# tsdconseil/libtsd

Hardware: AMD Instinct MI355X
Metric: Msamples/s, 127-tap FIR on 2^26 cfloat stream (higher is better)
Workload: dtype f32 (complex64 data, real f32 taps); 1 GPU; configs[1]: 127-tap FIR (design_rif_fen lp 0.02, real taps via filtrer()) on 2^26-sample Veccf per GPU, inputs resident in HBM; method=overlap-save, samples_per_gpu=67108864, pre_warm_steps=150, backend=none (one process, one GPU), world_size=1, self_launched=False

## Files before the change

### libtsd_amd/csrc/ols.hip

```cpp
#include "fir_internal.hpp"
#include "fft1024_wave.hpp"
#include <cstdlib>

namespace tsdgpu {

using namespace w1024;
constexpr int OLS_N = 1024;
#ifndef OLS_SCALAR
#define OLS_SCALAR 1
#endif
#ifndef OLS_RUN_DEFAULT
#define OLS_RUN_DEFAULT 2
#endif
#ifndef OLS_DYN_DEFAULT
#define OLS_DYN_DEFAULT 16
#endif
constexpr int OLS_MAX_CTR = 32;
#if OLS_SCALAR
using cv = cpx;
#else
using cv = v2f;
#endif
__device__ __forceinline__ cv mkv(float a, float b) { return Make<cv>::of(a, b); }

constexpr bool NT = false;
__device__ __forceinline__ cv ntload(const cv *p)
{
  v2f t = __builtin_nontemporal_load(reinterpret_cast<const v2f *>(p));
  return mkv(t.x, t.y);
}
__device__ __forceinline__ void ntstore(cv *p, cv v)
{
  v2f t = {v.x, v.y};
  __builtin_nontemporal_store(t, reinterpret_cast<v2f *>(p));
}
template <bool EDGE>
__device__ __forceinline__ void ols_fetch_real(cv (&v)[16], const float *__restrict__ x, const float *__restrict__ hist,
                                               int histlen, int Km1, int L, int64_t n, int64_t b, int lane)
{
  const int64_t ga = 2 * b * (int64_t) L - Km1, gb = ga + L;
  if (!EDGE) {
    const float *xa = x + ga, *xb = x + gb;
#pragma unroll
    for (int r = 0; r < 16; r++) v[r] = mkv(xa[64 * r + lane], xb[64 * r + lane]);
  } else {
#pragma unroll
    for (int r = 0; r < 16; r++) {
      const int64_t g1 = ga + 64 * r + lane, g2 = gb + 64 * r + lane;
      v[r] = mkv(g1 < 0 ? hist[histlen + g1] : (g1 < n ? x[g1] : 0.f), g2 < 0 ? hist[histlen + g2] : (g2 < n ? x[g2] : 0.f));
    }
  }
}
template <bool EDGE>
__device__ __forceinline__ void ols_fetch(cv (&v)[16], const cv *__restrict__ x, const cv *__restrict__ hist,
                                          int histlen, int Km1, int L, int64_t n, int64_t b, int lane)
{
  const int64_t g0 = b * (int64_t) L - Km1;
  if (!EDGE) {
    const cv *xb = x + g0;
#pragma unroll
    for (int r = 0; r < 16; r++) v[r] = NT ? ntload(xb + 64 * r + lane) : xb[64 * r + lane];
  } else {
#pragma unroll
    for (int r = 0; r < 16; r++) {
      const int64_t g = g0 + 64 * r + lane;
      v[r] = g < 0 ? hist[histlen + g] : (g < n ? x[g] : mkv(0.f, 0.f));
    }
  }
}

struct OlsDyn {
  unsigned *ctr;
  unsigned base, Q;
  int NC;
  int64_t nunits;
};
struct RegTab {
  cv v[16];
  __device__ __forceinline__ const cv &operator[](int r) const { return v[r]; }
};

template <bool EDGE, bool REAL, int R0, bool DYN>
__device__ __forceinline__ void ols_body(cv *lds, const void *__restrict__ xv, const void *__restrict__ histv,
                                         void *__restrict__ yv, const cv *__restrict__ Hreg,
                                         const cv *__restrict__ TW1, const cv *__restrict__ TW2, int Km1,
                                         int histlen, int L, int64_t n, int64_t b_lo, int64_t b_hi, int64_t G,
                                         int64_t w, int64_t cgrp, int R, OlsDyn dyn)
{
  const int lane = threadIdx.x & 63;
  const cv *x = (const cv *) xv, *hist = (const cv *) histv;
  cv *y = (cv *) yv;
  const float *xr = (const float *) xv, *histr = (const float *) histv;
  float *yr = (float *) yv;
  RegTab tw1r, tw2r, Hr;
#pragma unroll
  for (int r = 0; r < 16; r++) {
    tw1r.v[r] = TW1[r * 64 + lane];
    tw2r.v[r] = TW2[r * 64 + lane];
    Hr.v[r] = Hreg[r * 64 + lane];
  }
  auto sync = []() {
    __builtin_amdgcn_fence(__ATOMIC_RELEASE, "wavefront");
    __builtin_amdgcn_wave_barrier();
    __builtin_amdgcn_fence(__ATOMIC_ACQUIRE, "wavefront");
  };

  const int64_t slot = (G % 8 == 0) ? (w % 8) * (G / 8) + w / 8 : w;
  const int ctr_c = DYN ? (int) (cgrp % dyn.NC) : 0;
  auto pull_issue = [&]() -> unsigned {
    unsigned v = 0;
    if (lane == 0) v = __hip_atomic_fetch_add(dyn.ctr + ctr_c * 32, 1u, __ATOMIC_RELAXED, __HIP_MEMORY_SCOPE_AGENT);
    return v;
  };
  auto pull = [&]() -> int64_t {
    for (;;) {
      const unsigned v = (unsigned) __builtin_amdgcn_readfirstlane((int) pull_issue()) - dyn.base;
      if (v >= dyn.Q) return -1;
      const int64_t u = (int64_t) v * dyn.NC + ctr_c;
      if (u < dyn.nunits) return u;
    }
  };
  auto pull_finish = [&](unsigned raw) -> int64_t {
    const unsigned v = (unsigned) __builtin_amdgcn_readfirstlane((int) raw) - dyn.base;
    if (v >= dyn.Q) return -1;
    const int64_t u = (int64_t) v * dyn.NC + ctr_c;
    return u < dyn.nunits ? u : pull();
  };
  int64_t unit = EDGE ? 0 : (DYN ? pull() : slot);
  if (unit < 0) return;
  int64_t run0 = EDGE ? b_lo : b_lo + unit * R;
  int64_t b = run0;
  if (b >= b_hi) return;

  int64_t pulled = -1;
  auto process = [&](cv (&cur)[16], cv (&nxt)[16], int64_t blk, int64_t nb, bool inrun) {
    const bool more = !EDGE && nb < b_hi;
    cv keep[R0 > 0 ? R0 : 1], pre[R0 > 0 ? R0 : 1];
#pragma unroll
    for (int r = 0; r < R0; r++) keep[r] = cur[(16 - R0 + r) & 15];
    const int64_t pb = more ? nb : blk;
    if (!EDGE && R0 > 0) {
      if (!REAL) {
        const cv *xb = x + (pb * (int64_t) L - Km1);
        if (!inrun) {
#pragma unroll
          for (int r = 0; r < R0; r++) pre[r] = xb[64 * r + lane];
        }
#pragma unroll
        for (int r = R0; r < 16; r++) nxt[r] = NT ? ntload(xb + 64 * r + lane) : xb[64 * r + lane];
      } else {
        const float *xa = xr + (2 * pb * (int64_t) L - Km1), *xb = xa + L;
        if (!inrun) {
#pragma unroll
          for (int r = 0; r < R0; r++) pre[r] = mkv(xa[64 * r + lane], xb[64 * r + lane]);
        }
#pragma unroll
        for (int r = R0; r < 16; r++) nxt[r] = mkv(xa[64 * r + lane], xb[64 * r + lane]);
      }
    } else if (!EDGE) {
      if (REAL) ols_fetch_real<EDGE>(nxt, xr, histr, histlen, Km1, L, n, pb, lane);
      else ols_fetch<EDGE>(nxt, x, hist, histlen, Km1, L, n, pb, lane);
    }
    const bool pulls = DYN && more && !inrun;
    unsigned raw = 0;
    if (pulls) raw = pull_issue();
    forward(cur, lds, lane, tw1r, tw2r, sync);
#pragma unroll
    for (int r = 0; r < 16; r++) cur[r] = cmul(cur[r], Hr[r]);
    inverse(cur, lds, lane, tw1r, tw2r, sync);
    sync();
    if (!EDGE) {
#pragma unroll
      for (int r = R0; r < 16; r++) asm volatile("" ::"v"(nxt[r]));
#pragma unroll
      for (int r = 0; r < R0; r++) {
        asm volatile("" : "+v"(keep[r]));
        if (inrun) nxt[r] = REAL ? mkv(keep[r].y, nxt[(16 - R0 + r) & 15].x) : keep[r];
        else nxt[r] = pre[r];
      }
    }
    if (pulls) pulled = pull_finish(raw);
    const int r0 = (!EDGE && R0 > 0) ? R0 : Km1 >> 6;
    if (!REAL) {
      const int64_t o0 = blk * (int64_t) L;
      cv *yb = y + (o0 - Km1);
#pragma unroll
      for (int r = 0; r < 16; r++) {
        const int t = 64 * r + lane;
        if (!EDGE) {
          if (r >= r0) { if (NT) ntstore(yb + t, cur[r]); else yb[t] = cur[r]; }
        } else {
          if (r >= r0 && o0 + t - Km1 < n) yb[t] = cur[r];
        }
      }
    } else {
      const int64_t oa = 2 * blk * (int64_t) L, ob = oa + L;
      float *ya = yr + (oa - Km1), *yb = yr + (ob - Km1);
#pragma unroll
      for (int r = 0; r < 16; r++) {
        const int t = 64 * r + lane;
        if (!EDGE) {
          if (r >= r0) { ya[t] = cur[r].x; yb[t] = cur[r].y; }
        } else {
          if (r >= r0 && oa + t - Km1 < n) ya[t] = cur[r].x;
          if (r >= r0 && ob + t - Km1 < n) yb[t] = cur[r].y;
        }
      }
    }
  };

  cv A[16], B[16];
  if (REAL) ols_fetch_real<EDGE>(A, xr, histr, histlen, Km1, L, n, b, lane);
  else ols_fetch<EDGE>(A, x, hist, histlen, Km1, L, n, b, lane);
  if (EDGE) {
    process(A, B, b, b_hi, false);
    return;
  }
#pragma unroll
  for (int r = 0; r < 16; r++) asm volatile("" ::"v"(A[r]));
  int i = 0;
  constexpr int64_t END = INT64_MAX;
  auto unit_after = [&](int64_t u) -> int64_t {
    if (DYN) return pulled;
    return b_lo + (u + G) * R < b_hi ? u + G : -1;
  };
  int64_t unit_next = DYN ? pull() : unit_after(unit);
  auto next_of = [&](int64_t &nb, bool &inrun) {
    inrun = i + 1 < R && b + 1 < b_hi;
    nb = inrun ? b + 1 : (unit_next >= 0 ? b_lo + unit_next * R : END);
  };
  auto advance = [&](int64_t nb, bool inrun) {
    if (inrun) i++;
    else {
      i = 0;
      run0 = nb;
      unit = unit_next;
      unit_next = unit_after(unit);
    }
    b = nb;
  };
  for (;;) {
    int64_t nb;
    bool inrun;
    next_of(nb, inrun);
    process(A, B, b, nb, inrun);
    if (nb >= b_hi) break;
    advance(nb, inrun);
    next_of(nb, inrun);
    process(B, A, b, nb, inrun);
    if (nb >= b_hi) break;
    advance(nb, inrun);
  }
}

template <bool REAL, int R0, bool DYN>
__global__ __launch_bounds__(64, 2) void ols_kernel(const void *__restrict__ x, const void *__restrict__ hist,
                                                    void *__restrict__ hist_next, void *__restrict__ y,
                                                    const cpx *__restrict__ Hreg, const cpx *__restrict__ TW1,
                                                    const cpx *__restrict__ TW2, int Km1, int histlen, int L,
                                                    int64_t n, int64_t b_lo, int64_t b_hi, int64_t nblocks, int G,
                                                    int ne, int64_t n_lo, int64_t b_tail, int R, OlsDyn dyn)
{
  __shared__ cv lds[LDS_ELEMS];
  const int64_t w = (int64_t) blockIdx.x;
  const int lane = threadIdx.x & 63;
  if (w < G) {
    ols_body<false, REAL, R0, DYN>(lds, x, hist, y, (const cv *) Hreg, (const cv *) TW1, (const cv *) TW2, Km1, histlen, L, n, b_lo, b_hi, G,
                                       w, (int64_t) blockIdx.x / 8, R, dyn);
  } else if (w < G + ne) {
    const int64_t b = (w - G) < n_lo ? (int64_t) (w - G) : b_tail + (w - G - n_lo);
    ols_body<true, REAL, 0, false>(lds, x, hist, y, (const cv *) Hreg, (const cv *) TW1, (const cv *) TW2, Km1, histlen, L, n, b, nblocks, 1, 0, 0, 1, dyn);
  } else if (w == G + ne) {
    for (int i = lane; i < histlen; i += 64) {
      const int64_t g = n - histlen + i;
      if (REAL) ((float *) hist_next)[i] = g < 0 ? ((const float *) hist)[histlen + g] : ((const float *) x)[g];
      else ((cpx *) hist_next)[i] = g < 0 ? ((const cpx *) hist)[histlen + g] : ((const cpx *) x)[g];
    }
  }
}

bool ols_preferred(const tsdgpu_fir *f)
{
  if (ols_long_supported(f)) return true;
  if (f->data_type == TSDGPU_C64) return f->K >= (f->tap_type == TSDGPU_F32 ? 57 : 48) && f->K <= 513;
  return f->tap_type == TSDGPU_F32 && f->K >= 40 && f->K <= 513;
}

int ols_plan_create(tsdgpu_fir *f)
{
  if (ols_long_supported(f)) return ols_long_plan_create(f);
  if (f->K > OLS_N - 63) {
    f->method = TSDGPU_FIR_DIRECT;
    return TSDGPU_OK;
  }
  const int N = OLS_N, K = f->K;
  f->ols_N = N;
  f->ols_L = N - (int) (cdiv(K - 1, 64) * 64);
  std::vector<double> hr(K), hi(K, 0.0);
  if (f->tap_type == TSDGPU_F32) {
    const float *t = (const float *) f->taps_host.data();
    for (int i = 0; i < K; i++) hr[i] = t[i];
  } else {
    const float *t = (const float *) f->taps_host.data();
    for (int i = 0; i < K; i++) { hr[i] = t[2 * i]; hi[i] = t[2 * i + 1]; }
  }
  struct Tables {
    std::vector<double> c, s;
    std::vector<cpx> tw12;
    Tables() : c(OLS_N / 2), s(OLS_N / 2), tw12(2 * OLS_N)
    {
      const double PI = 3.14159265358979323846;
      for (int i = 0; i < OLS_N / 2; i++) { c[i] = std::cos(2 * PI * i / OLS_N); s[i] = -std::sin(2 * PI * i / OLS_N); }
      fill_twiddles(tw12.data(), tw12.data() + OLS_N);
    }
  };
  static const Tables *tb = new Tables();
  std::vector<double> ar(N, 0.0), ai(N, 0.0);
  int logn = 0;
  while ((1 << logn) < N) logn++;
  for (int i = 0; i < K; i++) {
    int rv = 0;
    for (int b = 0; b < logn; b++) rv |= ((i >> b) & 1) << (logn - 1 - b);
    ar[rv] = hr[i];
    ai[rv] = hi[i];
  }
  for (int len = 2; len <= N; len <<= 1) {
    const int half = len / 2, step = N / len;
    for (int base = 0; base < N; base += len)
      for (int j = 0; j < half; j++) {
        const double wr = tb->c[(size_t) j * step], wi = tb->s[(size_t) j * step];
        const int a = base + j, b = a + half;
        const double tr = ar[b] * wr - ai[b] * wi, ti = ar[b] * wi + ai[b] * wr;
        ar[b] = ar[a] - tr; ai[b] = ai[a] - ti;
        ar[a] += tr; ai[a] += ti;
      }
  }
  std::vector<cpx> img(3 * (size_t) N);
  for (int lane = 0; lane < 64; lane++)
    for (int r = 0; r < 16; r++) {
      const int k = freq_index(lane, r);
      img[r * 64 + lane] = mk((float) (ar[k] / N), (float) (ai[k] / N));
    }
  std::copy(tb->tw12.begin(), tb->tw12.end(), img.begin() + N);
  const size_t bytes = (size_t) N * sizeof(cpx);
  const size_t ctr_bytes = (size_t) OLS_MAX_CTR * 128;
  img.resize(3 * (size_t) N + ctr_bytes / sizeof(cpx), mk(0.f, 0.f));
  if (hipMalloc(&f->d_H, 3 * bytes + ctr_bytes) != hipSuccess)
    return set_err(TSDGPU_ERR_HIP, "ols: hipMalloc failed: %s", hipGetErrorString(hipGetLastError()));
  if (hipMemcpy(f->d_H, img.data(), 3 * bytes + ctr_bytes, hipMemcpyHostToDevice) != hipSuccess)
    return set_err(TSDGPU_ERR_HIP, "ols: upload failed: %s", hipGetErrorString(hipGetLastError()));
  f->d_ctr = (unsigned *) ((char *) f->d_H + 3 * bytes);
  f->ctr_base = 0;
  static const std::pair<int, int> occ = []() {
    int dev = 0, cus = 256, per_cu = 8;
    (void) hipGetDevice(&dev);
    (void) hipDeviceGetAttribute(&cus, hipDeviceAttributeMultiprocessorCount, dev);
    if (hipOccupancyMaxActiveBlocksPerMultiprocessor(&per_cu, ols_kernel<false, 2, true>, 64, 0) != hipSuccess || per_cu < 1) {
      (void) hipGetLastError();
      per_cu = 8;
    }
    return std::make_pair(cus, per_cu);
  }();
  const int cus = occ.first, per_cu = occ.second;
  f->ols_grid = cus * per_cu;
  if (getenv("TSDGPU_DEBUG")) fprintf(stderr, "[tsdgpu] ols plan: N=%d K=%d L=%d cus=%d waves/CU=%d grid=%d waves\n", N, K, f->ols_L, cus, per_cu, f->ols_grid);
  return TSDGPU_OK;
}

void ols_plan_destroy(tsdgpu_fir *f)
{
  if (f->d_H) (void) hipFree(f->d_H);
  f->d_H = nullptr;
  f->d_ctr = nullptr;
}

int ols_step(tsdgpu_fir *f, const void *x, void *y, int64_t n, hipStream_t st)
{
  const bool real = f->data_type == TSDGPU_F32;
  const int L = f->ols_L;
  const int64_t LB = real ? 2 * (int64_t) L : L;
  const int64_t nblocks = cdiv(n, LB);
  const cpx *d = (const cpx *) f->d_H;
  const int64_t ovl = OLS_N - L;
  const int64_t b_lo = std::min<int64_t>(nblocks, f->K > 1 ? cdiv(ovl, LB) : 0);
  const int64_t b_hi = std::max<int64_t>(b_lo, n / LB);
  int64_t grid = 0;
  const int r0 = (int) (ovl / 64);
  const char *run_s = dev_switch("OLS_RUN");
  const int run_env = run_s ? atoi(run_s) : OLS_RUN_DEFAULT;
  const char *nc_s = dev_switch("OLS_DYN");
  int NC = nc_s ? atoi(nc_s) : OLS_DYN_DEFAULT;
  if (NC < 0 || NC > OLS_MAX_CTR || f->capturable || !f->d_ctr || stream_is_capturing(st)) NC = 0;
  int R = 1;
  unsigned ctr_add = 0;
  OlsDyn dyn = {f->d_ctr, f->ctr_base, 0u, NC > 0 ? NC : 1, 0};
  if (b_hi > b_lo) {
    const int64_t nint = b_hi - b_lo;
    if (r0 >= 1 && r0 <= 4 && run_env > 1 && nint >= (int64_t) f->ols_grid * run_env * 2) R = run_env;
    const int64_t nruns = cdiv(nint, R);
    const char *min_s = dev_switch("OLS_DYN_MIN");
    const int64_t dyn_min = min_s ? atoi(min_s) : 4;
    if (NC > 0 && nruns >= dyn_min * (int64_t) f->ols_grid) {
      const int64_t grp = (int64_t) 8 * NC;
      grid = std::max<int64_t>(grp, (f->ols_grid / grp) * grp);
      if (NC != f->ctr_nc) {
        TSD_HIP(hipMemsetAsync(f->d_ctr, 0, (size_t) OLS_MAX_CTR * 128, st));
        f->ctr_base = 0;
        f->ctr_nc = NC;
        dyn.base = 0;
      }
      dyn.nunits = nruns;
      dyn.Q = (unsigned) cdiv(nruns, NC);
      ctr_add = dyn.Q + (unsigned) (grid / NC);
    } else {
      NC = 0;
      grid = nruns < f->ols_grid ? nruns : f->ols_grid;
      if (nruns > grid) {
        const int64_t rounds = cdiv(nruns, grid);
        grid = cdiv(cdiv(nruns, rounds), 8) * 8;
      }
    }
  } else NC = 0;
  const int64_t b_lo_w = b_lo;
  const int64_t n_lo = b_lo, b_tail = b_hi;
  const int ne = (int) (n_lo + (nblocks - b_tail));
  int64_t e[2] = {n_lo, b_tail};
  const int nxt = f->cur ^ 1;
  const unsigned nwg = (unsigned) (grid + ne + 1);
#define OLS_LAUNCH(REAL, R0, DYN)                                                                                                     \
  hipLaunchKernelGGL((ols_kernel<REAL, R0, DYN>), dim3(nwg), dim3(64), 0, st, x, (const void *) fir_hist_read(f),                        \
                     f->hist[nxt], y, d, d + OLS_N, d + 2 * OLS_N, OLS_N - L, f->HL, L, n, b_lo_w, b_hi, nblocks, (int) grid, ne,   \
                     e[0], e[1], R, dyn)
#define OLS_LAUNCH_R0(REAL, DYN)                                        \
  switch (R > 1 ? r0 : 0) {                                             \
    case 1: OLS_LAUNCH(REAL, 1, DYN); break;                            \
    case 2: OLS_LAUNCH(REAL, 2, DYN); break;                            \
    case 3: OLS_LAUNCH(REAL, 3, DYN); break;                            \
    case 4: OLS_LAUNCH(REAL, 4, DYN); break;                            \
    default: OLS_LAUNCH(REAL, 0, DYN); break;                           \
  }
  if (real) {
    if (NC > 0) { OLS_LAUNCH_R0(true, true) } else { OLS_LAUNCH_R0(true, false) }
  } else {
    if (NC > 0) { OLS_LAUNCH_R0(false, true) } else { OLS_LAUNCH_R0(false, false) }
  }
#undef OLS_LAUNCH_R0
#undef OLS_LAUNCH
  if (const hipError_t le = hipGetLastError(); le != hipSuccess) {
    if (NC > 0) f->ctr_nc = 0;
    return set_err(TSDGPU_ERR_HIP, "fir_step: overlap-save launch failed: %s", hipGetErrorString(le));
  }
  f->ctr_base += ctr_add;
  f->cur = nxt;
  return TSDGPU_OK;
}

__global__ __launch_bounds__(64, 2) void ola1024_kernel(const cpx *__restrict__ x, cpx *__restrict__ y, const cpx *__restrict__ Hreg,
                                                        const cpx *__restrict__ TW1, const cpx *__restrict__ TW2,
                                                        const cpx *__restrict__ svg_in, cpx *__restrict__ svg_out, int64_t B, int per)
{
  __shared__ cv lds[LDS_ELEMS];
  const int lane = threadIdx.x;
  const int64_t b_lo = (int64_t) blockIdx.x * per, b_hi = min(B, b_lo + (int64_t) per);
  if (b_lo >= B) return;
  cv tw1[16], tw2[16], H[16];
#pragma unroll
  for (int r = 0; r < 16; r++) {
    tw1[r] = ((const cv *) TW1)[r * 64 + lane];
    tw2[r] = ((const cv *) TW2)[r * 64 + lane];
    H[r] = ((const cv *) Hreg)[r * 64 + lane];
  }
  auto sync = []() {
    __builtin_amdgcn_fence(__ATOMIC_RELEASE, "wavefront");
    __builtin_amdgcn_wave_barrier();
    __builtin_amdgcn_fence(__ATOMIC_ACQUIRE, "wavefront");
  };
  const cv *xs = (const cv *) x;
  cv *ys = (cv *) y;
  cv cur[16], carry[8], nxt[8];
  auto transform = [&](cv (&v)[16]) {
    forward(v, lds, lane, tw1, tw2, sync);
#pragma unroll
    for (int r = 0; r < 16; r++) v[r] = cmul(v[r], H[r]);
    inverse(v, lds, lane, tw1, tw2, sync);
    sync();
  };
  if (b_lo == 0) {
#pragma unroll
    for (int r = 0; r < 8; r++) carry[r] = ((const cv *) svg_in)[64 * r + lane];
  } else {
#pragma unroll
    for (int r = 0; r < 8; r++) { cur[r] = mkv(0.f, 0.f); cur[8 + r] = xs[(b_lo - 1) * 512 + 64 * r + lane]; }
    transform(cur);
#pragma unroll
    for (int r = 0; r < 8; r++) carry[r] = cur[8 + r];
  }
#pragma unroll
  for (int r = 0; r < 8; r++) nxt[r] = xs[b_lo * 512 + 64 * r + lane];
  for (int64_t b = b_lo; b < b_hi; b++) {
#pragma unroll
    for (int r = 0; r < 8; r++) { cur[r] = mkv(0.f, 0.f); cur[8 + r] = nxt[r]; }
    const bool more = b + 1 < b_hi;
    if (more) {
#pragma unroll
      for (int r = 0; r < 8; r++) nxt[r] = xs[(b + 1) * 512 + 64 * r + lane];
    }
    transform(cur);
    if (more) {
#pragma unroll
      for (int r = 0; r < 8; r++) asm volatile("" ::"v"(nxt[r]));
    }
#pragma unroll
    for (int r = 0; r < 8; r++) {
      ys[b * 512 + 64 * r + lane] = mkv(cur[r].x + carry[r].x, cur[r].y + carry[r].y);
      carry[r] = cur[8 + r];
    }
  }
  if (b_hi == B) {
#pragma unroll
    for (int r = 0; r < 8; r++) ((cv *) svg_out)[64 * r + lane] = carry[r];
  }
}

void ola1024_tables(const cpx *H_host, cpx *out3)
{
  for (int lane = 0; lane < 64; lane++)
    for (int r = 0; r < 16; r++) {
      const cpx h = H_host[freq_index(lane, r)];
      out3[r * 64 + lane] = mk(h.x / 1024.f, h.y / 1024.f);
    }
  fill_twiddles(out3 + 1024, out3 + 2048);
}

int ola1024_launch(const cpx *x, cpx *y, const cpx *tables3, const cpx *svg_in, cpx *svg_out, int64_t B, hipStream_t st)
{
  if (B <= 0) return TSDGPU_OK;
  const int per = (int) std::min<int64_t>(16, std::max<int64_t>(1, cdiv(B, 2048)));
  const int64_t grid = cdiv(B, per);
  if (grid > 0x7fffffff) return set_err(TSDGPU_ERR_UNSUPPORTED, "ola: too many blocks in one call");
  hipLaunchKernelGGL(ola1024_kernel, dim3((unsigned) grid), dim3(64), 0, st, x, y, tables3, tables3 + 1024, tables3 + 2048, svg_in, svg_out, B, per);
  TSD_HIP(hipGetLastError());
  return TSDGPU_OK;
}

__global__ __launch_bounds__(64, 2) void olaw512_kernel(const cpx *__restrict__ blk0, int nrest, const cpx *__restrict__ x, cpx *__restrict__ y,
                                                        const cpx *__restrict__ Hreg, const cpx *__restrict__ TW1, const cpx *__restrict__ TW2,
                                                        const float *__restrict__ fen, const cpx *__restrict__ svg_in,
                                                        const cpx *__restrict__ last_in, const cpx *__restrict__ prev_half_in,
                                                        cpx *__restrict__ svg_out, cpx *__restrict__ last_out, int64_t B, int per,
                                                        int skip_first)
{
  __shared__ cv lds[LDS_ELEMS];
  const int lane = threadIdx.x;
  const int64_t b_lo = (int64_t) blockIdx.x * per, b_hi = min(B, b_lo + (int64_t) per);
  if (b_lo >= B) return;
  const int sig = (lane >> 1) & 1, c = 2 * (lane >> 2) + (lane & 1);
  cv tw1[16], tw2[16], H[8];
  float win[16];
#pragma unroll
  for (int r = 0; r < 16; r++) {
    tw1[r] = ((const cv *) TW1)[r * 64 + lane];
    tw2[r] = ((const cv *) TW2)[r * 64 + lane];
    win[r] = fen[32 * r + c];
  }
#pragma unroll
  for (int q = 0; q < 8; q++) H[q] = ((const cv *) Hreg)[q * 64 + lane];
  auto sync = []() {
    __builtin_amdgcn_fence(__ATOMIC_RELEASE, "wavefront");
    __builtin_amdgcn_wave_barrier();
    __builtin_amdgcn_fence(__ATOMIC_ACQUIRE, "wavefront");
  };
  auto sample = [&](int64_t i) -> cv {
    if (i < 0) return ((const cv *) prev_half_in)[i + 256];
    if (i < 512) return ((const cv *) blk0)[i];
    return ((const cv *) x)[i - nrest];
  };
  auto xchg = [&](cv a) -> cv {
    return mkv(__shfl_xor(a.x, 2), __shfl_xor(a.y, 2));
  };
  cv v[16], keep[8];
  int64_t p = b_lo <= 1 ? 0 : b_lo - 2;
  if (b_lo <= 1) {
#pragma unroll
    for (int r = 0; r < 8; r++) keep[r] = ((const cv *) svg_in)[256 + 32 * r + c];
    if (b_lo == 0 && !skip_first) {
#pragma unroll
      for (int r = 0; r < 8; r++) {
        const int i = 32 * r + c;
        cv o = ((const cv *) last_in)[256 * sig + i];
        if (sig) {
          const cv g = ((const cv *) svg_in)[i];
          o = mkv(o.x + g.x * 0.5f, o.y + g.y * 0.5f);
        }
        ((cv *) y)[256 * sig + i] = o;
      }
    }
  } else {
#pragma unroll
    for (int r = 0; r < 8; r++) keep[r] = mkv(0.f, 0.f);
  }
  const int64_t p_end = b_hi == B ? B : b_hi - 1;
  for (; p < p_end; p++) {
    const int64_t base = 512 * p - 256 + 256 * sig;
#pragma unroll
    for (int r = 0; r < 16; r++) {
      const cv a = sample(base + 32 * r + c);
      v[r] = mkv(a.x * win[r], a.y * win[r]);
    }
    forward_pair512(v, lds, lane, tw1, tw2, sync);
#pragma unroll
    for (int r = 0; r < 16; r++) v[r] = cmul(v[r], H[2 * (r >> 2) + (r & 1)]);
    inverse_pair512(v, lds, lane, tw1, tw2, sync);
    sync();
    cv got[8];
#pragma unroll
    for (int r = 0; r < 8; r++) got[r] = xchg(v[8 + r]);
    if (p + 1 < B) {
      if (p + 1 >= b_lo) {
        cv *yo = (cv *) y + (p + 1 - skip_first) * 512 + 256 * sig + c;
#pragma unroll
        for (int r = 0; r < 8; r++) {
          const cv o = sig ? got[r] : keep[r];
          yo[32 * r] = mkv(o.x * 0.5f + v[r].x * 0.5f, o.y * 0.5f + v[r].y * 0.5f);
        }
      }
    } else {
      if (sig) {
#pragma unroll
        for (int r = 0; r < 16; r++) ((cv *) svg_out)[32 * r + c] = v[r];
      } else {
#pragma unroll
        for (int r = 0; r < 8; r++) {
          ((cv *) last_out)[32 * r + c] = mkv(keep[r].x * 0.5f + v[r].x * 0.5f, keep[r].y * 0.5f + v[r].y * 0.5f);
          ((cv *) last_out)[256 + 32 * r + c] = mkv(v[8 + r].x * 0.5f, v[8 + r].y * 0.5f);
        }
      }
    }
#pragma unroll
    for (int r = 0; r < 8; r++) keep[r] = got[r];
  }
}

void olaw512_tables(const cpx *H_host, cpx *out)
{
  for (int lane = 0; lane < 64; lane++)
    for (int q = 0; q < 8; q++) {
      const cpx h = H_host[pair512_freq_index(lane, 4 * (q >> 1) + (q & 1))];
      out[q * 64 + lane] = mk(h.x / 512.f, h.y / 512.f);
    }
  fill_twiddles_pair512(out + 512, out + 512 + 1024);
}

int olaw512_launch(const cpx *blk0, int nrest, const cpx *x, cpx *y, const cpx *tables, const float *fen, const cpx *svg_in, const cpx *last_in,
                   const cpx *prev_half_in, cpx *svg_out, cpx *last_out, int64_t B, int skip_first, hipStream_t st)
{
  if (B <= 0) return TSDGPU_OK;
  const int per = (int) std::min<int64_t>(16, std::max<int64_t>(2, cdiv(B, 2048)));
  const int64_t grid = cdiv(B, per);
  if (grid > 0x7fffffff) return set_err(TSDGPU_ERR_UNSUPPORTED, "ola: too many blocks in one call");
  hipLaunchKernelGGL(olaw512_kernel, dim3((unsigned) grid), dim3(64), 0, st, blk0, nrest, x, y, tables, tables + 512, tables + 512 + 1024, fen, svg_in,
                     last_in, prev_half_in, svg_out, last_out, B, per, skip_first);
  TSD_HIP(hipGetLastError());
  return TSDGPU_OK;
}

__global__ __launch_bounds__(64, 2) void welch1024_kernel(const cpx *__restrict__ x, const float *__restrict__ w,
                                                          const cpx *__restrict__ TW1, const cpx *__restrict__ TW2,
                                                          float *__restrict__ part, int64_t nseg, int per)
{
  __shared__ cv lds[LDS_ELEMS];
  const int lane = threadIdx.x;
  const int64_t k_lo = (int64_t) blockIdx.x * per, k_hi = min(nseg, k_lo + (int64_t) per);
  cv tw1[16], tw2[16];
  float win[16], acc[16];
#pragma unroll
  for (int r = 0; r < 16; r++) {
    tw1[r] = ((const cv *) TW1)[r * 64 + lane];
    tw2[r] = ((const cv *) TW2)[r * 64 + lane];
    win[r] = w[64 * r + lane];
    acc[r] = 0.f;
  }
  auto sync = []() {
    __builtin_amdgcn_fence(__ATOMIC_RELEASE, "wavefront");
    __builtin_amdgcn_wave_barrier();
    __builtin_amdgcn_fence(__ATOMIC_ACQUIRE, "wavefront");
  };
  const cv *xs = (const cv *) x;
  cv cur[16], nxt[16];
  if (k_lo < k_hi) {
#pragma unroll
    for (int r = 0; r < 16; r++) nxt[r] = xs[k_lo * 512 + 64 * r + lane];
  }
  for (int64_t k = k_lo; k < k_hi; k++) {
#pragma unroll
    for (int r = 0; r < 16; r++) cur[r] = mkv(nxt[r].x * win[r], nxt[r].y * win[r]);
    if (k + 1 < k_hi) {
#pragma unroll
      for (int r = 0; r < 16; r++) nxt[r] = xs[(k + 1) * 512 + 64 * r + lane];
    }
    forward(cur, lds, lane, tw1, tw2, sync);
    sync();
#pragma unroll
    for (int r = 0; r < 16; r++) acc[r] += cur[r].x * cur[r].x + cur[r].y * cur[r].y;
  }
#pragma unroll
  for (int r = 0; r < 16; r++) part[(size_t) blockIdx.x * 1024 + ((freq_index(lane, r) + 512) & 1023)] = acc[r] * (1.0f / 1024.0f);
}

int welch1024_launch(const cpx *x, const float *w, const cpx *tw2x1024, float *part, int64_t nseg, int per, hipStream_t st)
{
  const int64_t grid = cdiv(nseg, per);
  hipLaunchKernelGGL(welch1024_kernel, dim3((unsigned) grid), dim3(64), 0, st, x, w, tw2x1024, tw2x1024 + 1024, part, nseg, per);
  TSD_HIP(hipGetLastError());
  return TSDGPU_OK;
}

void welch1024_tables(cpx *out2) { fill_twiddles(out2, out2 + 1024); }

}
```

Measured before the change: 335,400 Msamples/s.

## Pack four waves per workgroup and share filter spectrum in LDS

Launches four wavefronts per workgroup instead of one. The filter spectrum H is staged once into shared LDS, and the run-carry registers (keep) are spilled to per-wave LDS, which frees VGPRs so more waves fit per CU. Base pointers are forced into scalar registers to cut VALU address math, and the slot and counter-group mapping and grid rounding are adjusted for multi-wave groups. The cost is extra LDS traffic for the H multiply and the keep values, plus a __syncthreads at kernel start.

```diff
diff --git a/libtsd_amd/csrc/ols.hip b/libtsd_amd/csrc/ols.hip
--- a/libtsd_amd/csrc/ols.hip
+++ b/libtsd_amd/csrc/ols.hip
@@ -16,6 +16,7 @@
 #define OLS_DYN_DEFAULT 16
 #endif
 constexpr int OLS_MAX_CTR = 32;
+constexpr int OLS_W = 4;
 #if OLS_SCALAR
 using cv = cpx;
 #else
@@ -23,6 +24,13 @@
 #endif
 __device__ __forceinline__ cv mkv(float a, float b) { return Make<cv>::of(a, b); }
 
+template <typename T> __device__ __forceinline__ T *scalar_base(T *p)
+{
+  auto g = (__attribute__((address_space(1))) T *) p;
+  asm("" : "+s"(g));
+  return (T *) g;
+}
+
 constexpr bool NT = false;
 __device__ __forceinline__ cv ntload(const cv *p)
 {
@@ -40,7 +48,7 @@
 {
   const int64_t ga = 2 * b * (int64_t) L - Km1, gb = ga + L;
   if (!EDGE) {
-    const float *xa = x + ga, *xb = x + gb;
+    const float *xa = scalar_base(x + ga), *xb = scalar_base(x + gb);
 #pragma unroll
     for (int r = 0; r < 16; r++) v[r] = mkv(xa[64 * r + lane], xb[64 * r + lane]);
   } else {
@@ -57,7 +65,7 @@
 {
   const int64_t g0 = b * (int64_t) L - Km1;
   if (!EDGE) {
-    const cv *xb = x + g0;
+    const cv *xb = scalar_base(x + g0);
 #pragma unroll
     for (int r = 0; r < 16; r++) v[r] = NT ? ntload(xb + 64 * r + lane) : xb[64 * r + lane];
   } else {
@@ -81,23 +89,23 @@
 };
 
 template <bool EDGE, bool REAL, int R0, bool DYN>
-__device__ __forceinline__ void ols_body(cv *lds, const void *__restrict__ xv, const void *__restrict__ histv,
-                                         void *__restrict__ yv, const cv *__restrict__ Hreg,
+__device__ __forceinline__ void ols_body(cv *lds, const cv *hl, cv *kp, const void *__restrict__ xv,
+                                         const void *__restrict__ histv, void *__restrict__ yv,
                                          const cv *__restrict__ TW1, const cv *__restrict__ TW2, int Km1,
-                                         int histlen, int L, int64_t n, int64_t b_lo, int64_t b_hi, int64_t G,
-                                         int64_t w, int64_t cgrp, int R, OlsDyn dyn)
+                                         int histlen, int L, int64_t n, int64_t b_lo, int64_t b_end, int64_t G,
+                                         int64_t w, int xcd, int64_t cgrp, int R, OlsDyn dyn)
 {
   const int lane = threadIdx.x & 63;
+  int64_t b_hi = b_end;
   const cv *x = (const cv *) xv, *hist = (const cv *) histv;
   cv *y = (cv *) yv;
   const float *xr = (const float *) xv, *histr = (const float *) histv;
   float *yr = (float *) yv;
-  RegTab tw1r, tw2r, Hr;
+  RegTab tw1r, tw2r;
 #pragma unroll
   for (int r = 0; r < 16; r++) {
     tw1r.v[r] = TW1[r * 64 + lane];
     tw2r.v[r] = TW2[r * 64 + lane];
-    Hr.v[r] = Hreg[r * 64 + lane];
   }
   auto sync = []() {
     __builtin_amdgcn_fence(__ATOMIC_RELEASE, "wavefront");
@@ -105,7 +113,7 @@
     __builtin_amdgcn_fence(__ATOMIC_ACQUIRE, "wavefront");
   };
 
-  const int64_t slot = (G % 8 == 0) ? (w % 8) * (G / 8) + w / 8 : w;
+  const int64_t slot = (G % (8 * OLS_W) == 0) ? xcd * (G / 8) + cgrp : w;
   const int ctr_c = DYN ? (int) (cgrp % dyn.NC) : 0;
   auto pull_issue = [&]() -> unsigned {
     unsigned v = 0;
@@ -134,10 +142,11 @@
 
   int64_t pulled = -1;
   auto process = [&](cv (&cur)[16], cv (&nxt)[16], int64_t blk, int64_t nb, bool inrun) {
+    if (!EDGE) asm volatile("" : "+s"(b_hi));
     const bool more = !EDGE && nb < b_hi;
-    cv keep[R0 > 0 ? R0 : 1], pre[R0 > 0 ? R0 : 1];
-#pragma unroll
-    for (int r = 0; r < R0; r++) keep[r] = cur[(16 - R0 + r) & 15];
+    cv pre[R0 > 0 ? R0 : 1];
+#pragma unroll
+    for (int r = 0; r < R0; r++) kp[r * 64 + lane] = cur[(16 - R0 + r) & 15];
     const int64_t pb = more ? nb : blk;
     if (!EDGE && R0 > 0) {
       if (!REAL) {
@@ -166,7 +175,7 @@
     if (pulls) raw = pull_issue();
     forward(cur, lds, lane, tw1r, tw2r, sync);
 #pragma unroll
-    for (int r = 0; r < 16; r++) cur[r] = cmul(cur[r], Hr[r]);
+    for (int r = 0; r < 16; r++) cur[r] = cmul(cur[r], hl[r * 64 + lane]);
     inverse(cur, lds, lane, tw1r, tw2r, sync);
     sync();
     if (!EDGE) {
@@ -174,8 +183,8 @@
       for (int r = R0; r < 16; r++) asm volatile("" ::"v"(nxt[r]));
 #pragma unroll
       for (int r = 0; r < R0; r++) {
-        asm volatile("" : "+v"(keep[r]));
-        if (inrun) nxt[r] = REAL ? mkv(keep[r].y, nxt[(16 - R0 + r) & 15].x) : keep[r];
+        const cv keep = kp[r * 64 + lane];
+        if (inrun) nxt[r] = REAL ? mkv(keep.y, nxt[(16 - R0 + r) & 15].x) : keep;
         else nxt[r] = pre[r];
       }
     }
@@ -183,7 +192,7 @@
     const int r0 = (!EDGE && R0 > 0) ? R0 : Km1 >> 6;
     if (!REAL) {
       const int64_t o0 = blk * (int64_t) L;
-      cv *yb = y + (o0 - Km1);
+      cv *yb = EDGE ? y + (o0 - Km1) : scalar_base(y + (o0 - Km1));
 #pragma unroll
       for (int r = 0; r < 16; r++) {
         const int t = 64 * r + lane;
@@ -195,7 +204,7 @@
       }
     } else {
       const int64_t oa = 2 * blk * (int64_t) L, ob = oa + L;
-      float *ya = yr + (oa - Km1), *yb = yr + (ob - Km1);
+      float *ya = EDGE ? yr + (oa - Km1) : scalar_base(yr + (oa - Km1)), *yb = EDGE ? yr + (ob - Km1) : scalar_base(yr + (ob - Km1));
 #pragma unroll
       for (int r = 0; r < 16; r++) {
         const int t = 64 * r + lane;
@@ -254,22 +263,28 @@
 }
 
 template <bool REAL, int R0, bool DYN>
-__global__ __launch_bounds__(64, 2) void ols_kernel(const void *__restrict__ x, const void *__restrict__ hist,
-                                                    void *__restrict__ hist_next, void *__restrict__ y,
-                                                    const cpx *__restrict__ Hreg, const cpx *__restrict__ TW1,
-                                                    const cpx *__restrict__ TW2, int Km1, int histlen, int L,
-                                                    int64_t n, int64_t b_lo, int64_t b_hi, int64_t nblocks, int G,
-                                                    int ne, int64_t n_lo, int64_t b_tail, int R, OlsDyn dyn)
-{
-  __shared__ cv lds[LDS_ELEMS];
-  const int64_t w = (int64_t) blockIdx.x;
-  const int lane = threadIdx.x & 63;
+__global__ __launch_bounds__(64 * OLS_W, 3) void ols_kernel(const void *__restrict__ x, const void *__restrict__ hist,
+                                                            void *__restrict__ hist_next, void *__restrict__ y,
+                                                            const cpx *__restrict__ Hreg, const cpx *__restrict__ TW1,
+                                                            const cpx *__restrict__ TW2, int Km1, int histlen, int L,
+                                                            int64_t n, int64_t b_lo, int64_t b_hi, int64_t nblocks, int G,
+                                                            int ne, int64_t n_lo, int64_t b_tail, int R, OlsDyn dyn)
+{
+  constexpr int KEEP = 64 * R0;
+  __shared__ cv smem[OLS_W * LDS_ELEMS + OLS_N + OLS_W * KEEP];
+  const int wv = __builtin_amdgcn_readfirstlane((int) (threadIdx.x >> 6)), lane = threadIdx.x & 63;
+  cv *lds = smem + wv * LDS_ELEMS, *hl = smem + OLS_W * LDS_ELEMS, *kp = hl + OLS_N + wv * KEEP;
+  for (int i = threadIdx.x; i < OLS_N; i += 64 * OLS_W) hl[i] = ((const cv *) Hreg)[i];
+  __syncthreads();
+  const int64_t w = (int64_t) blockIdx.x * OLS_W + wv;
+  const int xcd = (int) (blockIdx.x % 8);
+  const int64_t cgrp = (int64_t) (blockIdx.x / 8) * OLS_W + wv;
   if (w < G) {
-    ols_body<false, REAL, R0, DYN>(lds, x, hist, y, (const cv *) Hreg, (const cv *) TW1, (const cv *) TW2, Km1, histlen, L, n, b_lo, b_hi, G,
-                                       w, (int64_t) blockIdx.x / 8, R, dyn);
+    ols_body<false, REAL, R0, DYN>(lds, hl, kp, x, hist, y, (const cv *) TW1, (const cv *) TW2, Km1, histlen, L, n, b_lo, b_hi, G,
+                                       w, xcd, cgrp, R, dyn);
   } else if (w < G + ne) {
     const int64_t b = (w - G) < n_lo ? (int64_t) (w - G) : b_tail + (w - G - n_lo);
-    ols_body<true, REAL, 0, false>(lds, x, hist, y, (const cv *) Hreg, (const cv *) TW1, (const cv *) TW2, Km1, histlen, L, n, b, nblocks, 1, 0, 0, 1, dyn);
+    ols_body<true, REAL, 0, false>(lds, hl, kp, x, hist, y, (const cv *) TW1, (const cv *) TW2, Km1, histlen, L, n, b, nblocks, 1, 0, 0, 0, 1, dyn);
   } else if (w == G + ne) {
     for (int i = lane; i < histlen; i += 64) {
       const int64_t g = n - histlen + i;
@@ -352,18 +367,20 @@
   f->d_ctr = (unsigned *) ((char *) f->d_H + 3 * bytes);
   f->ctr_base = 0;
   static const std::pair<int, int> occ = []() {
-    int dev = 0, cus = 256, per_cu = 8;
+    int dev = 0, cus = 256, per_cu = 3;
     (void) hipGetDevice(&dev);
     (void) hipDeviceGetAttribute(&cus, hipDeviceAttributeMultiprocessorCount, dev);
-    if (hipOccupancyMaxActiveBlocksPerMultiprocessor(&per_cu, ols_kernel<false, 2, true>, 64, 0) != hipSuccess || per_cu < 1) {
+    if (hipOccupancyMaxActiveBlocksPerMultiprocessor(&per_cu, ols_kernel<false, 2, true>, 64 * OLS_W, 0) != hipSuccess || per_cu < 1) {
       (void) hipGetLastError();
-      per_cu = 8;
+      per_cu = 3;
     }
     return std::make_pair(cus, per_cu);
   }();
   const int cus = occ.first, per_cu = occ.second;
-  f->ols_grid = cus * per_cu;
-  if (getenv("TSDGPU_DEBUG")) fprintf(stderr, "[tsdgpu] ols plan: N=%d K=%d L=%d cus=%d waves/CU=%d grid=%d waves\n", N, K, f->ols_L, cus, per_cu, f->ols_grid);
+  f->ols_grid = cus * per_cu * OLS_W;
+  if (getenv("TSDGPU_DEBUG"))
+    fprintf(stderr, "[tsdgpu] ols plan: N=%d K=%d L=%d cus=%d workgroups/CU=%d waves/workgroup=%d grid=%d waves\n", N, K, f->ols_L, cus, per_cu,
+            OLS_W, f->ols_grid);
   return TSDGPU_OK;
 }
 
@@ -401,7 +418,9 @@
     const char *min_s = dev_switch("OLS_DYN_MIN");
     const int64_t dyn_min = min_s ? atoi(min_s) : 4;
     if (NC > 0 && nruns >= dyn_min * (int64_t) f->ols_grid) {
-      const int64_t grp = (int64_t) 8 * NC;
+      int64_t m = NC;
+      while (m % OLS_W) m += NC;
+      const int64_t grp = 8 * m;
       grid = std::max<int64_t>(grp, (f->ols_grid / grp) * grp);
       if (NC != f->ctr_nc) {
         TSD_HIP(hipMemsetAsync(f->d_ctr, 0, (size_t) OLS_MAX_CTR * 128, st));
@@ -417,7 +436,7 @@
       grid = nruns < f->ols_grid ? nruns : f->ols_grid;
       if (nruns > grid) {
         const int64_t rounds = cdiv(nruns, grid);
-        grid = cdiv(cdiv(nruns, rounds), 8) * 8;
+        grid = cdiv(cdiv(nruns, rounds), 8 * OLS_W) * (8 * OLS_W);
       }
     }
   } else NC = 0;
@@ -426,9 +445,9 @@
   const int ne = (int) (n_lo + (nblocks - b_tail));
   int64_t e[2] = {n_lo, b_tail};
   const int nxt = f->cur ^ 1;
-  const unsigned nwg = (unsigned) (grid + ne + 1);
+  const unsigned nwg = (unsigned) cdiv(grid + ne + 1, (int64_t) OLS_W);
 #define OLS_LAUNCH(REAL, R0, DYN)                                                                                                     \
-  hipLaunchKernelGGL((ols_kernel<REAL, R0, DYN>), dim3(nwg), dim3(64), 0, st, x, (const void *) fir_hist_read(f),                        \
+  hipLaunchKernelGGL((ols_kernel<REAL, R0, DYN>), dim3(nwg), dim3(64 * OLS_W), 0, st, x, (const void *) fir_hist_read(f),                \
                      f->hist[nxt], y, d, d + OLS_N, d + 2 * OLS_N, OLS_N - L, f->HL, L, n, b_lo_w, b_hi, nblocks, (int) grid, ne,   \
                      e[0], e[1], R, dyn)
 #define OLS_LAUNCH_R0(REAL, DYN)                                        \
```

Result: slower. 321,100 Msamples/s (-4.3%).
